# KohakuBlueleaf/UwUDiff

Hardware: AMD Instinct MI355X
Metric: train images/sec (whole node), DiT-S/2 256^2 latent (higher is better)
Workload: dtype bf16; 1 GPU; DiT-S/2 (L12 D384 h6), 4x32x32 synthetic latents + pooled-text cond 1280, eps-MSE, AdamW lr1e-6 wd0.01 cosine; random-init weights; per_gpu_batch=768, global_batch=768, parallelism=dp1

## Files before the change

include/uwu_hip.h:

```cpp
#ifndef UWU_HIP_H
#define UWU_HIP_H

#include <stddef.h>
#include <stdint.h>

#ifdef __cplusplus
extern "C" {
#endif

#define UWU_F32 0
#define UWU_BF16 1

#define UWU_OK 0
#define UWU_EINVAL (-1)
#define UWU_ELAUNCH (-2)
#define UWU_ENOTIMPL (-3)

#define UWU_PT_EPSILON 0
#define UWU_PT_V 1
#define UWU_PT_SAMPLE 2
#define UWU_PT_RF 3

#define UWU_EPI_NONE 0
#define UWU_EPI_BIAS 1
// ... 138 lines not shown
enum {
  UWU_PROF_GEMM_FWD = 0, UWU_PROF_GEMM_DGRAD = 1, UWU_PROF_GEMM_WGRAD = 2, UWU_PROF_GEMM_FC1_GELU = 3,
  UWU_PROF_GEMM_FC2_DGELU = 4, UWU_PROF_ATTN_FWD = 5, UWU_PROF_ATTN_BWD = 6, UWU_PROF_LN_FWD = 7, UWU_PROF_LN_BWD = 8,
  UWU_PROF_CONV = 9, UWU_PROF_OTHER = 10
};
int uwu_prof_enable(int on);
int uwu_prof_collect(int tag, int kind, double* ms, double* flops, double* bytes, int* launches);

int uwu_colsum(const void* X, int dtype, int M, int N, int ldx, float* out, int accumulate, void* stream);

int uwu_skinny_linear_ok(int M, int N, int K);
int uwu_skinny_linear_fwd(const float* X, const float* W, const float* bias, float* Y, float* Y2, int M, int N, int K,
                          int epilogue, void* stream);
int uwu_skinny_linear_dgrad(const float* dY, const float* W, float* dX, int M, int N, int K, void* stream);
int uwu_skinny_linear_wgrad(const float* dY, const float* X, float* dW, float* db, int M, int N, int K, void* stream);
int uwu_colsum_batched(const void* X, int dtype, int batch, int M, int N, int ldx, float* out, int accumulate,
                       void* stream);


int uwu_add_ln_modulate_fwd(const void* x_in, const void* y, const float* gate, const float* shift,
                            const float* scale, int mod_ld, void* x_out, void* h, float* mean, float* rstd,
                            int B, int T, int D, float eps, int affine, int dtype, void* stream);
int uwu_add_ln_modulate_fwd_q8(const void* x_in, const void* y, const float* gate, const float* shift, const float* scale,
                               int mod_ld, void* x_out, void* q8, int ldq, void* q8t, int ldqt, const float* q_scale,
                               float* q_amax, float* mean, float* rstd, int B, int T, int D, float eps, void* stream);


int uwu_add_ln_modulate_bwd(const void* dh, const void* x, const float* mean, const float* rstd,
                            const float* scale, const void* dx_in, const void* y, const float* gate,
                            int mod_ld, void* dx_out, void* dy, float* dshift, float* dscale, float* dgate,
// ... 43 lines not shown
int uwu_attention_rope_fwd(const void* q, const void* k, const void* v, const float* rope_tab, void* o, float* lse, int B,
                           int T, int H, int d, int ldq, int ldk, int ldv, int ldo, int ldt, float scale, int dtype,
                           void* stream);
int uwu_attention_rope_bwd(const void* q, const void* k, const void* v, const float* rope_tab, const void* o, const void* dO,
                           const float* lse, void* dq, void* dk, void* dv, int B, int T, int H, int d, int ldq, int ldk,
                           int ldv, int ldo, int ldt, float scale, int dtype, void* stream);


int uwu_timestep_embedding(const float* t, int B, int dim, float max_period, void* out, int dtype,
                           void* stream);
int uwu_silu_fwd(const void* x, void* y, int64_t n, int dtype, void* stream);
int uwu_silu_bwd(const void* x, const void* dy, void* dx, int64_t n, int dtype, void* stream);

int uwu_add(const void* a, const void* b, void* out, int64_t n, int dtype, void* stream);
int uwu_transpose_bf16(const void* src, void* dst, int rows, int cols, int ld_src, int ld_dst, void* stream);

int uwu_patchify(const float* img, void* tok, int B, int C, int H, int W, int p, int dtype, void* stream);
int uwu_unpatchify(const void* tok, int dtype, float* img, int B, int C, int H, int W, int p, void* stream);
int uwu_add_pos(void* x, const float* pos, int B, int T, int D, int dtype, void* stream);


int uwu_groupnorm_fwd(const void* x, const float* gamma, const float* beta, void* y, float* mean, float* rstd,
                      int B, int HW, int C, int G, float eps, int silu, int dtype, void* stream);
size_t uwu_groupnorm_fwd_det_ws_bytes(int B, int HW, int C, int G);
int uwu_groupnorm_fwd_det(const void* x, const float* gamma, const float* beta, void* y, float* mean, float* rstd, void* ws,
                          size_t ws_bytes, int B, int HW, int C, int G, float eps, int silu, int dtype, void* stream);
int uwu_groupnorm_bwd(const void* dy, const void* x, const float* mean, const float* rstd, const float* gamma,
                      const float* beta, void* dx, float* dgamma, float* dbeta, float* ws, int B, int HW, int C, int G,
                      int silu, int dtype, void* stream);
int uwu_im2col3x3(const void* x, void* col, int B, int H, int W, int C, int stride, int dtype, void* stream);
// ... 46 lines not shown
```

uwudiff_amd/csrc/dit.cpp:

```cpp
#include <hip/hip_runtime.h>
#include <math.h>
#include <stddef.h>
#include <stdint.h>
#include <stdlib.h>

#include "../../include/uwu_hip.h"
#include "env.h"

void uwu_set_error(const char* fmt, ...);

namespace {

constexpr int WGRAD_BLOCKS = 512;

struct Layout {
  size_t es;
  int64_t M, D, D3, D4, Kp, Ko;
  size_t feat, t_pre, t_h, temb, yemb, c, sc, mod;
  size_t sc16, dmod16;
  size_t tok, xe;
  size_t layer0, layer_stride;
  bool ckpt;
  size_t keep, scratch0;
  size_t o_x0, o_m1, o_r1, o_h1, o_qkv, o_lse, o_ao, o_y1, o_x1, o_m2, o_r2, o_h2, o_u, o_f, o_y2;
  size_t o_rope;
  size_t o_h1t, o_aot, o_h2t, o_ft;
  size_t xF, mF, rF, hF, otok;
  size_t dx, dy, dh, dqkv, dao, du, delta, dotok, dmod, dsc, dc, dth, dtp;
  size_t w2t;
  size_t wsc, wsc_bytes;
  size_t x8, x8t, dy8, dy8t, w8, w8_layer;
  size_t total;
};

inline size_t al(size_t x) { return (x + 255) & ~(size_t)255; }

Layout make_layout(const uwu_dit_desc& d) {
  Layout L{};
  L.es = d.dtype == UWU_BF16 ? 2 : 4;
  L.M = (int64_t)d.B * d.T;
  L.D = d.D;
  L.D3 = 3 * (int64_t)d.D;
  L.D4 = (int64_t)d.mlp_ratio * d.D;
  L.Kp = (int64_t)d.in_ch * d.patch * d.patch;
  L.Ko = (int64_t)d.out_ch * d.patch * d.patch;
  size_t p = 0;
  auto take = [&](size_t bytes) { size_t o = p; p = al(p + bytes); return o; };
  const size_t f4 = 4;
  L.feat = take((size_t)d.B * d.freq_dim * f4);
  L.t_pre = take((size_t)d.B * d.D * f4);
// ... 36 lines not shown
  L.layer_stride = L.ckpt ? L.keep : q;
  L.layer0 = p;
  p += (size_t)d.L * L.layer_stride;
  if (L.ckpt) L.scratch0 = take(q);
  L.xF = take(L.M * L.D * L.es);
  L.mF = take(L.M * f4);
  L.rF = take(L.M * f4);
  L.hF = take(L.M * L.D * L.es);
  L.otok = take(L.M * L.Ko * L.es);
  L.dx = take(L.M * L.D * L.es);
  L.dy = take(L.M * L.D * L.es);
  L.dh = take(L.M * L.D * L.es);
  L.dqkv = take(L.M * L.D3 * L.es);
  L.dao = take(L.M * L.D * L.es);
  L.du = take(L.M * L.D4 * L.es);
  L.w2t = take((size_t)L.D4 * d.D * 2);
  L.delta = take((size_t)d.B * d.H * d.T * f4);
  L.dotok = take(L.M * L.Ko * L.es);
  L.dmod = take((size_t)d.B * d.mod_total * f4);
  L.dsc = take((size_t)d.B * d.D * f4);
  L.dc = take((size_t)d.B * d.D * f4);
  L.dth = take((size_t)d.B * d.D * f4);
  L.dtp = take((size_t)d.B * d.D * f4);
  L.wsc_bytes = uwu_gemm_wgrad_scratch_bytes((int)L.D4, d.D, (int)L.M);
  for (const size_t t : {uwu_gemm_wgrad_scratch_bytes(d.D, (int)L.D4, (int)L.M),
                         uwu_gemm_wgrad_scratch_bytes((int)L.D3, d.D, (int)L.M),
                         uwu_gemm_wgrad_scratch_bytes(d.D, d.D, (int)L.M),
                         uwu_gemm_wgrad_pair_scratch_bytes((int)L.D4, d.D, d.D, (int)L.D4, (int)L.M),
                         uwu_gemm_wgrad_pair_scratch_bytes((int)L.D3, d.D, d.D, d.D, (int)L.M)})
    if (t > L.wsc_bytes) L.wsc_bytes = t;
  if (d.fp8) {
// ... 39 lines not shown
    if (d->fp8 < 0 || d->fp8 > 2 || d->dtype != UWU_BF16 || d->D % 128 || d->mlp_ratio != 4 || ((int64_t)d->B * d->T) % 128 ||
        !d->f8_scale || !d->f8_amax || !d->f8_fmt) {
      uwu_set_error("dit: fp8 mode needs bf16 activations, D %% 128 == 0, B*T %% 128 == 0, mlp_ratio 4 and the scale / amax / fmt arrays");
      return UWU_EINVAL;
    }
  }
  return UWU_OK;
}

#define RUN(expr)              \
  do {                         \
    int rc_ = (expr);          \
    if (rc_ != UWU_OK) return rc_; \
  } while (0)

int lin_fwd(const void* X, const void* W, const float* bias, void* Y, void* Y2, int M, int N, int K, int dt, int cdt,
            int epi, void* st) {
  return uwu_gemm(X, W, Y, Y2, bias, nullptr, M, N, K, K, K, N, 0, 0, 0, dt, cdt, epi, 1, st);
}
int lin_fwd32(const float* X, const float* W, const float* bias, float* Y, float* Y2, int M, int N, int K, int epi, void* st) {
  if (M <= 16 && N <= 4096 && uwu_skinny_linear_ok(M, N, K)) return uwu_skinny_linear_fwd(X, W, bias, Y, Y2, M, N, K, epi, st);
  return lin_fwd(X, W, bias, Y, Y2, M, N, K, UWU_F32, UWU_F32, epi, st);
}
int lin_dgrad(const void* dY, const void* W, void* dX, const void* aux, int M, int N, int K, int dt, void* st,
              float* colsum = nullptr) {
  return uwu_gemm(dY, W, dX, colsum, nullptr, aux, M, K, N, N, K, K, K, 0, 1, dt, dt,
                  aux ? UWU_EPI_DGELU : UWU_EPI_NONE, 1, st);
}
static bool mod_bf16(const uwu_dit_desc& d) {
  return d.dtype == UWU_BF16 && d.B >= 64 && d.mod_total % 8 == 0;
}
int lin_dgrad_splitk(const void* dY, const void* W, float* dX, int M, int N, int K, void* st) {
  if (hipMemsetAsync(dX, 0, (size_t)M * K * sizeof(float), (hipStream_t)st) != hipSuccess) {
    uwu_set_error("dgrad_splitk: memset failed");
    return UWU_ELAUNCH;
  }
// ... 20 lines not shown
  if (split > ktiles) split = ktiles;
  if (split < 1) split = 1;
  return uwu_gemm(dY, X, dW, nullptr, nullptr, nullptr, N, K, M, N, K, K, 0, 1, 1, dt, UWU_F32, UWU_EPI_ACCUM, split, st);
}

bool wgrad_pair_ok(int M, int Na, int Ka, int Nb, int Kb, size_t scratch_bytes) {
  const size_t need = uwu_gemm_wgrad_pair_scratch_bytes(Na, Ka, Nb, Kb, M);
  return need && need <= scratch_bytes;
}
int lin_wgrad_pair(const void* dYa, const void* Xa, float* dWa, float* dba, int Na, int Ka, const void* dYb, const void* Xb,
                   float* dWb, float* dbb, int Nb, int Kb, int M, void* st, void* scratch, size_t scratch_bytes) {
  return uwu_gemm_wgrad_pair(dYa, Xa, dWa, dba, Na, Ka, Na, Ka, Ka, dYb, Xb, dWb, dbb, Nb, Kb, Nb, Kb, Kb, M, UWU_BF16,
                             WGRAD_BLOCKS, scratch, scratch_bytes, st);
}

int lin_wgrad32(const float* dY, const float* X, float* dW, float* db, int M, int N, int K, void* st) {
  if (M <= 16 && uwu_skinny_linear_ok(M, N, K)) return uwu_skinny_linear_wgrad(dY, X, dW, db, M, N, K, st);
  RUN(lin_wgrad(dY, X, dW, M, N, K, UWU_F32, st));
  return uwu_colsum(dY, UWU_F32, M, N, N, db, 1, st);
}

struct F8 {
  int mode;
  float* scale;
  float* amax;
  const int32_t* fmt;
  char *x8, *x8t, *dy8, *dy8t, *wsc, *w8;
  size_t wsc_bytes, w8_layer;
  int D;
  void* st;
  int role(int l, int r) const { return 12 * l + r; }
  char* w(int l, int i, bool t) const {
// ... 250 lines not shown
  RUN(uwu_timestep_embedding(t, B, d.freq_dim, 10000.f, P.at(L.feat), UWU_F32, st));
  RUN(lin_fwd32(P.at<float>(L.feat), w32 + d.off_t_w1, w32 + d.off_t_b1, P.at<float>(L.t_pre), P.at<float>(L.t_h), B, D,
                d.freq_dim, UWU_EPI_BIAS_SILU, st));
  RUN(lin_fwd32(P.at<float>(L.t_h), w32 + d.off_t_w2, w32 + d.off_t_b2, P.at<float>(L.temb), nullptr, B, D, D, UWU_EPI_BIAS, st));
  const void* cptr = P.at(L.temb);
  if (cond) {
    RUN(lin_fwd32(cond, w32 + d.off_y_w, w32 + d.off_y_b, P.at<float>(L.yemb), nullptr, B, D, d.cond_dim, UWU_EPI_BIAS, st));
    RUN(uwu_add(P.at(L.temb), P.at(L.yemb), P.at(L.c), (int64_t)B * D, UWU_F32, st));
    cptr = P.at(L.c);
  }
  RUN(uwu_silu_fwd(cptr, P.at(L.sc), (int64_t)B * D, UWU_F32, st));
  if (mod_bf16(d)) {
    RUN(uwu_cast_f32_to_bf16(P.at<float>(L.sc), P.at(L.sc16), (int64_t)B * D, st));
    RUN(lin_fwd(P.at(L.sc16), wb + d.off_mod_w * es, w32 + d.off_mod_b, P.at(L.mod), nullptr, B, ML, D, UWU_BF16, UWU_F32, UWU_EPI_BIAS, st));
  } else {
    RUN(lin_fwd32(P.at<float>(L.sc), w32 + d.off_mod_w, w32 + d.off_mod_b, P.at<float>(L.mod), nullptr, B, ML, D, UWU_EPI_BIAS, st));
  }
  const float* mod = P.at<float>(L.mod);

  const F8 f8{d.fp8, d.f8_scale, d.f8_amax, d.f8_fmt, P.at<char>(L.x8), nullptr, P.at<char>(L.dy8),
              P.at<char>(L.dy8t), P.at<char>(L.wsc), P.at<char>(L.w8), L.wsc_bytes, L.w8_layer, d.D, st};
  if (d.fp8) {
    const F8 fw{2, d.f8_scale, d.f8_amax, d.f8_fmt, nullptr, nullptr, nullptr, nullptr, nullptr, f8.w8, 0, L.w8_layer, d.D, st};
    const int rows[4] = {D3, D, D4, D}, cols[4] = {D, D, D, D4};
    for (int l = 0; l < d.L; ++l) {
      const LayerW w = layer_weights(d, l);
      const void* ws4[4] = {w.qkv_w, w.o_w, w.fc1_w, w.fc2_w};
      for (int i = 0; i < 4; ++i)
        RUN(uwu_fp8_amax(ws4[i], UWU_BF16, (int64_t)rows[i] * cols[i], d.f8_amax + fw.role(l, 8 + i), st));
    }
    RUN(uwu_fp8_update_scales(d.f8_amax, d.f8_scale, d.f8_fmt, 12 * d.L, 1.f, st));
    for (int l = 0; l < d.L; ++l) {
      const LayerW w = layer_weights(d, l);
      const void* ws4[4] = {w.qkv_w, w.o_w, w.fc1_w, w.fc2_w};
      for (int i = 0; i < 4; ++i)
        RUN(fw.quant(ws4[i], UWU_BF16, rows[i], cols[i], fw.role(l, 8 + i), fw.w(l, i, false), fw.w(l, i, true), nullptr, true));
    }
  }

  RUN(uwu_patchify(noisy, P.at(L.tok), B, d.in_ch, d.img, d.img, d.patch, dt, st));
  RUN(lin_fwd(P.at(L.tok), wb + d.off_patch_w * es, w32 + d.off_patch_b, P.lay(0, L.o_x0), nullptr, M, D, (int)L.Kp, dt,
              dt, UWU_EPI_BIAS, st));
  RUN(uwu_add_pos(P.lay(0, L.o_x0), d.pos, B, T, D, dt, st));

  for (int l = 0; l < d.L; ++l) RUN(block_forward(d, L, P, f8, l, false, st));
  {
    const int l = d.L - 1;
    const float* mp = mod + (int64_t)l * 6 * D;
    const float* mf = mod + (int64_t)d.L * 6 * D;
    RUN(uwu_add_ln_modulate_fwd(P.lay(l, L.o_x1), P.lay(l, L.o_y2), mp + 5 * D, mf + 0, mf + D, ML, P.at(L.xF),
                                P.at(L.hF), P.at<float>(L.mF), P.at<float>(L.rF), B, T, D, d.ln_eps, 0, dt, st));
    RUN(lin_fwd(P.at(L.hF), wb + d.off_final_w * es, w32 + d.off_final_b, P.at(L.otok), nullptr, M, (int)L.Ko, D, dt, dt,
                UWU_EPI_BIAS, st));
    RUN(uwu_unpatchify(P.at(L.otok), dt, out, B, d.out_ch, d.img, d.img, d.patch, st));
  }
  return UWU_OK;
}

// ... 15 lines not shown
  if (hipMemsetAsync(dmod, 0, (size_t)B * ML * sizeof(float), (hipStream_t)st) != hipSuccess) {
    uwu_set_error("dit_backward: memset failed");
    return UWU_ELAUNCH;
  }
  const float scale = 1.f / sqrtf((float)(D / d.H));
  const F8 f8{d.fp8, d.f8_scale, d.f8_amax, d.f8_fmt, P.at<char>(L.x8), nullptr, P.at<char>(L.dy8),
              P.at<char>(L.dy8t), P.at<char>(L.wsc), P.at<char>(L.w8), L.wsc_bytes, L.w8_layer, d.D, st};
  Fork fk{static_cast<hipStream_t>(st), {}, {}, false};
  fk.on = d.side_stream && d.side_stream != st && !d.fp8 && dt == UWU_BF16 && M <= 16384 && !L.ckpt &&
          fork_resources(fk, static_cast<hipStream_t>(d.side_stream));
  char* const wsc = P.at<char>(L.wsc);
  bool side_used[4] = {false, false, false, false};
  const bool pairs = !fk.on && !d.fp8 && dt == UWU_BF16 && M > 16384 && !L.ckpt;
  const bool pair_fc = pairs && wgrad_pair_ok(M, D4, D, D, D4, L.wsc_bytes);
  const bool pair_attn = pairs && wgrad_pair_ok(M, D3, D, D, D, L.wsc_bytes);

  RUN(uwu_patchify(dout, P.at(L.dotok), B, d.out_ch, d.img, d.img, d.patch, dt, st));
  RUN(lin_wgrad(P.at(L.dotok), P.at(L.hF), g + d.off_final_w, M, (int)L.Ko, D, dt, st));
  RUN(uwu_colsum(P.at(L.dotok), dt, M, (int)L.Ko, (int)L.Ko, g + d.off_final_b, 1, st));
  RUN(lin_dgrad(P.at(L.dotok), wb + d.off_final_w * es, P.at(L.dh), nullptr, M, (int)L.Ko, D, dt, st));
  {
    const int l = d.L - 1;
    const float* mp = mod + (int64_t)l * 6 * D;
    const float* mf = mod + (int64_t)d.L * 6 * D;
    float* dmp = dmod + (int64_t)l * 6 * D;
    float* dmf = dmod + (int64_t)d.L * 6 * D;
    RUN(uwu_add_ln_modulate_bwd(P.at(L.dh), P.at(L.xF), P.at<float>(L.mF), P.at<float>(L.rF), mf + D, nullptr,
                                P.lay(l, L.o_y2), mp + 5 * D, ML, P.at(L.dx), P.at(L.dy), dmf + 0, dmf + D, dmp + 5 * D,
                                B, T, D, 0, dt, st));
  }
// ... 9 lines not shown
                   f8.role(l, 6), f8.role(l, 2), f8.role(l, 10), f8.x8, f8.dy8t));
      } else {
      RUN(f8_bwd(f8, P.at(L.dy), P.lay(l, L.o_ft), f8.w(l, 3, true), g + w.off_fc2_w, g + w.off_fc2_b, P.at(L.du), P.lay(l, L.o_u),
                 g + w.off_fc1_b, M, D, D4, f8.role(l, 7), f8.role(l, 3), f8.role(l, 11)));
      RUN(f8_bwd(f8, P.at(L.du), P.lay(l, L.o_h2t), f8.w(l, 2, true), g + w.off_fc1_w, nullptr, P.at(L.dh), nullptr, nullptr, M, D4, D,
                 f8.role(l, 6), f8.role(l, 2), f8.role(l, 10)));
      }
    } else {
    if (!pair_fc) {
    RUN(on_side(fk, 0, [&](void* s2, int k) {
      return lin_wgrad(P.at(L.dy), P.lay(l, L.o_f), g + w.off_fc2_w, M, D, D4, dt, s2, wsc + (size_t)k * L.wsc_bytes, L.wsc_bytes, g + w.off_fc2_b);
    }));
    side_used[0] = true;
    }
    if (side_used[1]) RUN(join_side(fk, 1));
    if (dt == UWU_BF16 && D == 384 && M % 256 == 0 && M >= 256 * 256 && D4 % 64 == 0 && D4 >= 1024 && D4 <= 2048) {
      RUN(uwu_transpose_bf16(w.fc2_w, P.at(L.w2t), D, D4, D4, D, st));
      RUN(uwu_gemm(P.at(L.dy), P.at(L.w2t), P.at(L.du), nullptr, nullptr, P.lay(l, L.o_u), M, D4, D, D, D, D4, D4, 0, 0, dt, dt,
                   UWU_EPI_DGELU, 1, st));
    } else {
      RUN(lin_dgrad(P.at(L.dy), w.fc2_w, P.at(L.du), P.lay(l, L.o_u), M, D, D4, dt, st, nullptr));
    }
    if (pair_fc) {
      RUN(lin_wgrad_pair(P.at(L.du), P.lay(l, L.o_h2), g + w.off_fc1_w, g + w.off_fc1_b, D4, D, P.at(L.dy), P.lay(l, L.o_f),
                         g + w.off_fc2_w, g + w.off_fc2_b, D, D4, M, st, wsc, L.wsc_bytes));
    } else {
    RUN(on_side(fk, 1, [&](void* s2, int k) {
      return lin_wgrad(P.at(L.du), P.lay(l, L.o_h2), g + w.off_fc1_w, M, D4, D, dt, s2, wsc + (size_t)k * L.wsc_bytes, L.wsc_bytes, g + w.off_fc1_b);
    }));
    side_used[1] = true;
    }
    RUN(lin_dgrad(P.at(L.du), w.fc1_w, P.at(L.dh), nullptr, M, D4, D, dt, st));
    RUN(join_side(fk, 0));
// ... 75 lines not shown
    RUN(uwu_cast_f32_to_bf16(dmod, P.at(L.dmod16), (int64_t)B * ML, st));
    RUN(lin_wgrad(P.at(L.dmod16), P.at(L.sc16), g + d.off_mod_w, B, ML, D, UWU_BF16, st));
    RUN(uwu_colsum(dmod, UWU_F32, B, ML, ML, g + d.off_mod_b, 1, st));
    if (hipMemsetAsync(P.at(L.dsc), 0, (size_t)B * D * sizeof(float), (hipStream_t)st) != hipSuccess) {
      uwu_set_error("dit_backward: memset failed");
      return UWU_ELAUNCH;
    }
    {
      const int tiles = ((B + 127) / 128) * ((D + 127) / 128), ktiles = (ML + 63) / 64;
      int split = (512 + tiles - 1) / tiles;
      if (split > ktiles) split = ktiles;
      RUN(uwu_gemm(P.at(L.dmod16), wb + d.off_mod_w * es, P.at(L.dsc), nullptr, nullptr, nullptr, B, D, ML, ML, D, D, 0, 0, 1, UWU_BF16,
                   UWU_F32, UWU_EPI_ACCUM, split, st));
    }
  } else {
    RUN(lin_wgrad32(dmod, P.at<float>(L.sc), g + d.off_mod_w, g + d.off_mod_b, B, ML, D, st));
    RUN(lin_dgrad_splitk(dmod, w32 + d.off_mod_w, P.at<float>(L.dsc), B, ML, D, st));
  }
  const void* cptr = d.cond_dim > 0 ? P.at(L.c) : P.at(L.temb);
  RUN(uwu_silu_bwd(cptr, P.at(L.dsc), P.at(L.dc), (int64_t)B * D, UWU_F32, st));
  if (d.cond_dim > 0) {
  }
  RUN(lin_wgrad32(P.at<float>(L.dc), P.at<float>(L.t_h), g + d.off_t_w2, g + d.off_t_b2, B, D, D, st));
  if (B <= 16 && uwu_skinny_linear_ok(B, D, D) && D <= 512) RUN(uwu_skinny_linear_dgrad(P.at<float>(L.dc), w32 + d.off_t_w2, P.at<float>(L.dth), B, D, D, st));
  else RUN(lin_dgrad(P.at(L.dc), w32 + d.off_t_w2, P.at(L.dth), nullptr, B, D, D, UWU_F32, st));
  RUN(uwu_silu_bwd(P.at(L.t_pre), P.at(L.dth), P.at(L.dtp), (int64_t)B * D, UWU_F32, st));
  RUN(lin_wgrad32(P.at<float>(L.dtp), P.at<float>(L.feat), g + d.off_t_w1, g + d.off_t_b1, B, D, d.freq_dim, st));
  return UWU_OK;
}

extern "C" int uwu_dit_backward_cond(const uwu_dit_desc* dp, const float* cond, void* st) {
  RUN(check_desc(dp));
  const uwu_dit_desc& d = *dp;
  if (d.cond_dim <= 0) return UWU_OK;
  if (!cond || !d.g32) { uwu_set_error("dit_backward_cond: null tensor"); return UWU_EINVAL; }
  const Layout L = make_layout(d);
  Ptrs P{static_cast<char*>(d.ws), L};
  return lin_wgrad32(P.at<float>(L.dc), cond, d.g32 + d.off_y_w, d.g32 + d.off_y_b, d.B, d.D, d.cond_dim, st);
}
// ... 1 lines not shown
```

uwudiff_amd/lib.py:

```python
import ctypes
import os
from ctypes import c_char_p, c_float, c_int, c_int32, c_int64, c_size_t, c_void_p

import torch

_HERE = os.path.dirname(os.path.abspath(__file__))
LIB_PATH = os.path.join(_HERE, "libuwu_hip.so")

F32, BF16 = 0, 1
PT = {"epsilon": 0, "v_prediction": 1, "sample": 2, "rectified_flow": 3}
EPI_NONE, EPI_BIAS, EPI_BIAS_GELU, EPI_DGELU, EPI_BIAS_SILU, EPI_ACCUM = 0, 1, 2, 3, 4, 5
ACT = {"quick_gelu": 0, "gelu": 1}
GATE = {"gated-gelu": 0}


class UwuError(RuntimeError):
    pass


class DitDesc(ctypes.Structure):
    _fields_ = (
        [(n, c_int32) for n in ("B", "T", "D", "H", "L", "mlp_ratio", "in_ch", "out_ch", "patch", "img", "dtype",
                                "cond_dim", "freq_dim")]
        + [("ln_eps", c_float), ("mod_total", c_int32)]
# ... 63 lines not shown
                                  P, P]),
    "uwu_gemm_wgrad_scratch_bytes": (ctypes.c_size_t, [c_int, c_int, c_int]),
    "uwu_gemm_wgrad": (c_int, [P, P, P, P] + [c_int] * 8 + [P, ctypes.c_size_t, P]),
    "uwu_gemm_wgrad_pair_scratch_bytes": (ctypes.c_size_t, [c_int] * 5),
    "uwu_gemm_wgrad_pair": (c_int, ([P, P, P, P] + [c_int] * 5) * 2 + [c_int] * 3 + [P, ctypes.c_size_t, P]),
    "uwu_gemm_prof_enable": (c_int, [c_int]),
    "uwu_gemm_prof_collect": (c_int, [c_int, P, P, P]),
    "uwu_prof_enable": (c_int, [c_int]),
    "uwu_prof_collect": (c_int, [c_int, c_int, P, P, P, P]),
    "uwu_colsum": (c_int, [P, c_int, c_int, c_int, c_int, P, c_int, P]),
    "uwu_colsum_batched": (c_int, [P, c_int, c_int, c_int, c_int, c_int, P, c_int, P]),
    "uwu_skinny_linear_ok": (c_int, [c_int, c_int, c_int]),
    "uwu_skinny_linear_fwd": (c_int, [P, P, P, P, P, c_int, c_int, c_int, c_int, P]),
    "uwu_skinny_linear_dgrad": (c_int, [P, P, P, c_int, c_int, c_int, P]),
    "uwu_skinny_linear_wgrad": (c_int, [P, P, P, P, c_int, c_int, c_int, P]),
    "uwu_add_ln_modulate_fwd": (c_int, [P, P, P, P, P, c_int, P, P, P, P, c_int, c_int, c_int, c_float, c_int, c_int, P]),
    "uwu_add_ln_modulate_fwd_q8": (c_int, [P, P, P, P, P, c_int, P, P, c_int, P, c_int, P, P, P, P, c_int, c_int, c_int, c_float, P]),
    "uwu_add_ln_modulate_bwd": (c_int, [P, P, P, P, P, P, P, P, c_int, P, P, P, P, P, c_int, c_int, c_int, c_int, c_int, P]),
    "uwu_attention_fwd": (c_int, [P, P, P, P, P] + [c_int] * 9 + [c_float, c_int, P]),
    "uwu_attention_d512_fwd": (c_int, [P, P, P, P] + [c_int] * 6 + [c_float, c_int, P]),
    "uwu_attention_causal_fwd": (c_int, [P] * 5 + [c_int] * 8 + [c_float, c_int, P]),
    "uwu_text_embed": (c_int, [P, P, P, P, c_int, c_int, c_int, c_int, c_int, P]),
    "uwu_bias_act_fwd": (c_int, [P, P, P, c_int, c_int, c_int, c_int, c_int, P]),
    "uwu_text_pool": (c_int, [P, P, P, c_int, c_int, c_int, c_int, c_int, P]),
    "uwu_attention_relbias_fwd": (c_int, [P] * 6 + [c_int] * 8 + [c_float, c_int, P]),
    "uwu_add_rmsnorm_fwd": (c_int, [P] * 5 + [c_int, c_int, c_float, c_int, P]),
    "uwu_gated_act_fwd": (c_int, [P, P] + [c_int] * 6 + [P]),
    "uwu_t5_rel_bias": (c_int, [P, P, P, c_int, c_int, c_int, P]),
    "uwu_token_embed": (c_int, [P, P, P, c_int, c_int, c_int, c_int, c_int, P]),
    "uwu_attention_bwd": (c_int, [P] * 10 + [c_int] * 9 + [c_float, c_int, P]),
# ... 100 lines not shown
```

Baseline: 17640 images/s.

## Add edge kernels for patch embed, small fp32 linears, and batched fc2 transpose

```diff
diff --git a/include/uwu_hip.h b/include/uwu_hip.h
--- a/include/uwu_hip.h
+++ b/include/uwu_hip.h
@@ -176,6 +176,14 @@
                           int epilogue, void* stream);
 int uwu_skinny_linear_dgrad(const float* dY, const float* W, float* dX, int M, int N, int K, void* stream);
 int uwu_skinny_linear_wgrad(const float* dY, const float* X, float* dW, float* db, int M, int N, int K, void* stream);
+int uwu_edge_patch_ok(int D, int Kp);
+int uwu_edge_patch_fwd(const void* tok, const void* W, const float* bias, const float* pos, void* x0, int B, int T, int D,
+                       int Kp, void* stream);
+int uwu_edge_linear_ok(int M, int N, int K);
+int uwu_edge_linear_fwd(const float* X, const float* W, const float* bias, float* Y, float* Y2, int M, int N, int K,
+                        int epilogue, void* stream);
+int uwu_edge_linear_wgrad(const float* dY, const float* X, float* dW, float* db, int M, int N, int K, void* stream);
+int uwu_edge_linear_dgrad(const float* dY, const float* W, float* dX, int M, int N, int K, void* stream);
 int uwu_colsum_batched(const void* X, int dtype, int batch, int M, int N, int ldx, float* out, int accumulate,
                        void* stream);
 
@@ -249,6 +257,8 @@
 
 int uwu_add(const void* a, const void* b, void* out, int64_t n, int dtype, void* stream);
 int uwu_transpose_bf16(const void* src, void* dst, int rows, int cols, int ld_src, int ld_dst, void* stream);
+int uwu_transpose_bf16_batched(const void* src, void* dst, int rows, int cols, int ld_src, int ld_dst, int batch,
+                               int64_t stride_src, int64_t stride_dst, void* stream);
 
 int uwu_patchify(const float* img, void* tok, int B, int C, int H, int W, int p, int dtype, void* stream);
 int uwu_unpatchify(const void* tok, int dtype, float* img, int B, int C, int H, int W, int p, void* stream);
diff --git a/uwudiff_amd/csrc/dit.cpp b/uwudiff_amd/csrc/dit.cpp
--- a/uwudiff_amd/csrc/dit.cpp
+++ b/uwudiff_amd/csrc/dit.cpp
@@ -27,6 +27,7 @@
   size_t o_h1t, o_aot, o_h2t, o_ft;
   size_t xF, mF, rF, hF, otok;
   size_t dx, dy, dh, dqkv, dao, du, delta, dotok, dmod, dsc, dc, dth, dtp;
+  int w2t_layers;
   size_t w2t;
   size_t wsc, wsc_bytes;
   size_t x8, x8t, dy8, dy8t, w8, w8_layer;
@@ -34,6 +35,10 @@
 };
 
 inline size_t al(size_t x) { return (x + 255) & ~(size_t)255; }
+
+inline bool w2t_shape(const uwu_dit_desc& d, int64_t M, int64_t D4) {
+  return !d.fp8 && d.dtype == UWU_BF16 && d.D == 384 && M % 256 == 0 && M >= 256 * 256 && D4 % 64 == 0 && D4 >= 1024 && D4 <= 2048;
+}
 
 Layout make_layout(const uwu_dit_desc& d) {
   Layout L{};
@@ -100,7 +105,8 @@
   L.dqkv = take(L.M * L.D3 * L.es);
   L.dao = take(L.M * L.D * L.es);
   L.du = take(L.M * L.D4 * L.es);
-  L.w2t = take((size_t)L.D4 * d.D * 2);
+  L.w2t_layers = w2t_shape(d, L.M, L.D4) && !d.checkpoint ? d.L : 1;
+  L.w2t = take((size_t)L.w2t_layers * L.D4 * d.D * 2);
   L.delta = take((size_t)d.B * d.H * d.T * f4);
   L.dotok = take(L.M * L.Ko * L.es);
   L.dmod = take((size_t)d.B * d.mod_total * f4);
@@ -170,12 +176,20 @@
     if (rc_ != UWU_OK) return rc_; \
   } while (0)
 
+inline bool al16(const void* p) { return (reinterpret_cast<uintptr_t>(p) & 15) == 0; }
+static bool edge_on() {
+  static UwuEnv off("UWU_DIT_EDGE");
+  return !off.get().is('0');
+}
+
 int lin_fwd(const void* X, const void* W, const float* bias, void* Y, void* Y2, int M, int N, int K, int dt, int cdt,
             int epi, void* st) {
   return uwu_gemm(X, W, Y, Y2, bias, nullptr, M, N, K, K, K, N, 0, 0, 0, dt, cdt, epi, 1, st);
 }
-int lin_fwd32(const float* X, const float* W, const float* bias, float* Y, float* Y2, int M, int N, int K, int epi, void* st) {
+int lin_fwd32(const float* X, const float* W, const float* bias, float* Y, float* Y2, int M, int N, int K, int epi, void* st,
+              bool rows = true) {
   if (M <= 16 && N <= 4096 && uwu_skinny_linear_ok(M, N, K)) return uwu_skinny_linear_fwd(X, W, bias, Y, Y2, M, N, K, epi, st);
+  if (rows && M > 16 && edge_on() && uwu_edge_linear_ok(M, N, K) && al16(X)) return uwu_edge_linear_fwd(X, W, bias, Y, Y2, M, N, K, epi, st);
   return lin_fwd(X, W, bias, Y, Y2, M, N, K, UWU_F32, UWU_F32, epi, st);
 }
 int lin_dgrad(const void* dY, const void* W, void* dX, const void* aux, int M, int N, int K, int dt, void* st,
@@ -226,8 +240,9 @@
                              WGRAD_BLOCKS, scratch, scratch_bytes, st);
 }
 
-int lin_wgrad32(const float* dY, const float* X, float* dW, float* db, int M, int N, int K, void* st) {
+int lin_wgrad32(const float* dY, const float* X, float* dW, float* db, int M, int N, int K, void* st, bool rows = true) {
   if (M <= 16 && uwu_skinny_linear_ok(M, N, K)) return uwu_skinny_linear_wgrad(dY, X, dW, db, M, N, K, st);
+  if (rows && M > 16 && edge_on() && uwu_edge_linear_ok(M, N, K) && al16(X)) return uwu_edge_linear_wgrad(dY, X, dW, db, M, N, K, st);
   RUN(lin_wgrad(dY, X, dW, M, N, K, UWU_F32, st));
   return uwu_colsum(dY, UWU_F32, M, N, N, db, 1, st);
 }
@@ -508,7 +523,8 @@
     RUN(uwu_cast_f32_to_bf16(P.at<float>(L.sc), P.at(L.sc16), (int64_t)B * D, st));
     RUN(lin_fwd(P.at(L.sc16), wb + d.off_mod_w * es, w32 + d.off_mod_b, P.at(L.mod), nullptr, B, ML, D, UWU_BF16, UWU_F32, UWU_EPI_BIAS, st));
   } else {
-    RUN(lin_fwd32(P.at<float>(L.sc), w32 + d.off_mod_w, w32 + d.off_mod_b, P.at<float>(L.mod), nullptr, B, ML, D, UWU_EPI_BIAS, st));
+    RUN(lin_fwd32(P.at<float>(L.sc), w32 + d.off_mod_w, w32 + d.off_mod_b, P.at<float>(L.mod), nullptr, B, ML, D, UWU_EPI_BIAS, st,
+                  false));
   }
   const float* mod = P.at<float>(L.mod);
 
@@ -533,9 +549,13 @@
   }
 
   RUN(uwu_patchify(noisy, P.at(L.tok), B, d.in_ch, d.img, d.img, d.patch, dt, st));
-  RUN(lin_fwd(P.at(L.tok), wb + d.off_patch_w * es, w32 + d.off_patch_b, P.lay(0, L.o_x0), nullptr, M, D, (int)L.Kp, dt,
-              dt, UWU_EPI_BIAS, st));
-  RUN(uwu_add_pos(P.lay(0, L.o_x0), d.pos, B, T, D, dt, st));
+  if (dt == UWU_BF16 && edge_on() && uwu_edge_patch_ok(D, (int)L.Kp)) {
+    RUN(uwu_edge_patch_fwd(P.at(L.tok), wb + d.off_patch_w * es, w32 + d.off_patch_b, d.pos, P.lay(0, L.o_x0), B, T, D, (int)L.Kp, st));
+  } else {
+    RUN(lin_fwd(P.at(L.tok), wb + d.off_patch_w * es, w32 + d.off_patch_b, P.lay(0, L.o_x0), nullptr, M, D, (int)L.Kp, dt,
+                dt, UWU_EPI_BIAS, st));
+    RUN(uwu_add_pos(P.lay(0, L.o_x0), d.pos, B, T, D, dt, st));
+  }
 
   for (int l = 0; l < d.L; ++l) RUN(block_forward(d, L, P, f8, l, false, st));
   {
@@ -581,6 +601,11 @@
   const bool pairs = !fk.on && !d.fp8 && dt == UWU_BF16 && M > 16384 && !L.ckpt;
   const bool pair_fc = pairs && wgrad_pair_ok(M, D4, D, D, D4, L.wsc_bytes);
   const bool pair_attn = pairs && wgrad_pair_ok(M, D3, D, D, D, L.wsc_bytes);
+
+  const bool w2t_path = w2t_shape(d, M, D4);
+  const bool w2t_once = w2t_path && edge_on() && L.w2t_layers == d.L;
+  if (w2t_once)
+    RUN(uwu_transpose_bf16_batched(layer_weights(d, 0).fc2_w, P.at(L.w2t), D, D4, D4, D, d.L, d.layer_stride, (int64_t)D4 * D, st));
 
   RUN(uwu_patchify(dout, P.at(L.dotok), B, d.out_ch, d.img, d.img, d.patch, dt, st));
   RUN(lin_wgrad(P.at(L.dotok), P.at(L.hF), g + d.off_final_w, M, (int)L.Ko, D, dt, st));
@@ -620,9 +645,10 @@
     side_used[0] = true;
     }
     if (side_used[1]) RUN(join_side(fk, 1));
-    if (dt == UWU_BF16 && D == 384 && M % 256 == 0 && M >= 256 * 256 && D4 % 64 == 0 && D4 >= 1024 && D4 <= 2048) {
-      RUN(uwu_transpose_bf16(w.fc2_w, P.at(L.w2t), D, D4, D4, D, st));
-      RUN(uwu_gemm(P.at(L.dy), P.at(L.w2t), P.at(L.du), nullptr, nullptr, P.lay(l, L.o_u), M, D4, D, D, D, D4, D4, 0, 0, dt, dt,
+    if (w2t_path) {
+      const void* w2t = P.at<char>(L.w2t) + (w2t_once ? (size_t)l * D4 * D * 2 : 0);
+      if (!w2t_once) RUN(uwu_transpose_bf16(w.fc2_w, P.at(L.w2t), D, D4, D4, D, st));
+      RUN(uwu_gemm(P.at(L.dy), w2t, P.at(L.du), nullptr, nullptr, P.lay(l, L.o_u), M, D4, D, D, D, D4, D4, 0, 0, dt, dt,
                    UWU_EPI_DGELU, 1, st));
     } else {
       RUN(lin_dgrad(P.at(L.dy), w.fc2_w, P.at(L.du), P.lay(l, L.o_u), M, D, D4, dt, st, nullptr));
@@ -728,7 +754,7 @@
                    UWU_F32, UWU_EPI_ACCUM, split, st));
     }
   } else {
-    RUN(lin_wgrad32(dmod, P.at<float>(L.sc), g + d.off_mod_w, g + d.off_mod_b, B, ML, D, st));
+    RUN(lin_wgrad32(dmod, P.at<float>(L.sc), g + d.off_mod_w, g + d.off_mod_b, B, ML, D, st, false));
     RUN(lin_dgrad_splitk(dmod, w32 + d.off_mod_w, P.at<float>(L.dsc), B, ML, D, st));
   }
   const void* cptr = d.cond_dim > 0 ? P.at(L.c) : P.at(L.temb);
@@ -737,6 +763,7 @@
   }
   RUN(lin_wgrad32(P.at<float>(L.dc), P.at<float>(L.t_h), g + d.off_t_w2, g + d.off_t_b2, B, D, D, st));
   if (B <= 16 && uwu_skinny_linear_ok(B, D, D) && D <= 512) RUN(uwu_skinny_linear_dgrad(P.at<float>(L.dc), w32 + d.off_t_w2, P.at<float>(L.dth), B, D, D, st));
+  else if (edge_on() && uwu_edge_linear_ok(B, D, D)) RUN(uwu_edge_linear_dgrad(P.at<float>(L.dc), w32 + d.off_t_w2, P.at<float>(L.dth), B, D, D, st));
   else RUN(lin_dgrad(P.at(L.dc), w32 + d.off_t_w2, P.at(L.dth), nullptr, B, D, D, UWU_F32, st));
   RUN(uwu_silu_bwd(P.at(L.t_pre), P.at(L.dth), P.at(L.dtp), (int64_t)B * D, UWU_F32, st));
   RUN(lin_wgrad32(P.at<float>(L.dtp), P.at<float>(L.feat), g + d.off_t_w1, g + d.off_t_b1, B, D, d.freq_dim, st));
diff --git a/uwudiff_amd/csrc/edge.hip b/uwudiff_amd/csrc/edge.hip
--- /dev/null
+++ b/uwudiff_amd/csrc/edge.hip
@@ -0,0 +1,249 @@
+#include "common.h"
+
+namespace {
+
+__device__ __forceinline__ int feat_of_row(int r) { return (r & 16) | ((r & 4) << 1) | ((r & 8) >> 1) | (r & 3); }
+
+template <int NKS, bool POS>
+__global__ void __launch_bounds__(256) edge_patch_fwd_kernel(const bf16_t* __restrict__ tok, const bf16_t* __restrict__ W,
+                                                             const float* __restrict__ bias, const float* __restrict__ pos,
+                                                             bf16_t* __restrict__ x0, int B, int T, int D, int Kp, int bblocks) {
+  const int lane = threadIdx.x & 63, r = lane & 31, h = lane >> 5;
+  const int nwaves = gridDim.x * 4;
+  const int ntiles = T * bblocks, nblocks = (D + 31) >> 5;
+  const int frow = feat_of_row(r);
+  const uint4 zero4 = {0u, 0u, 0u, 0u};
+  for (int tile = blockIdx.x * 4 + (threadIdx.x >> 6); tile < ntiles; tile += nwaves) {
+    const int bb = tile / T, t = tile - bb * T;
+    const int b = bb * 32 + r;
+    const bool live = b < B;
+    const int64_t m = (int64_t)(live ? b : B - 1) * T + t;
+    uint4 tf[NKS];
+#pragma unroll
+    for (int ks = 0; ks < NKS; ++ks) {
+      const int k0 = ks * 16 + 8 * h;
+      tf[ks] = k0 < Kp ? *reinterpret_cast<const uint4*>(tok + m * Kp + k0) : zero4;
+    }
+    for (int nb = 0; nb < nblocks; ++nb) {
+      const int feat = nb * 32 + frow;
+      f32x16 acc;
+#pragma unroll
+      for (int i = 0; i < 16; ++i) acc[i] = 0.f;
+#pragma unroll
+      for (int ks = 0; ks < NKS; ++ks) {
+        const int k0 = ks * 16 + 8 * h;
+        const uint4 wf = (feat < D && k0 < Kp) ? *reinterpret_cast<const uint4*>(W + (int64_t)feat * Kp + k0) : zero4;
+        acc = __builtin_amdgcn_mfma_f32_32x32x16_bf16(*reinterpret_cast<const bf16x8*>(&wf),
+                                                      *reinterpret_cast<const bf16x8*>(&tf[ks]), acc, 0, 0, 0);
+      }
+#pragma unroll
+      for (int g = 0; g < 2; ++g) {
+        const int f0 = nb * 32 + g * 16 + h * 8;
+        if (f0 < D && live) {
+          const f32x8 bv = load8(bias + f0);
+          f32x8 v;
+#pragma unroll
+          for (int j = 0; j < 8; ++j) v[j] = (float)(bf16_t)(acc[8 * g + j] + bv[j]);
+          if (POS) v = v + load8(pos + (int64_t)t * D + f0);
+          store8(x0 + m * D + f0, v);
+        }
+      }
+    }
+  }
+}
+
+enum { LIN_FWD = 0, LIN_WGRAD = 1, LIN_DGRAD = 2 };
+constexpr int LT = 32, LLD = 36;
+
+template <bool TR>
+__device__ __forceinline__ f32x4 lin_tile_load(const float* __restrict__ G, int idx0, int nidx, int c0, int nc, int ld, int tid) {
+  const int a = tid >> 3, q = (tid & 7) * 4;
+  const int gi = TR ? idx0 + a : idx0 + q, gc = TR ? c0 + q : c0 + a;
+  if (gi >= nidx || gc >= nc) return f32x4{0.f, 0.f, 0.f, 0.f};
+  return load4(TR ? G + (int64_t)gi * ld + gc : G + (int64_t)gc * ld + gi);
+}
+template <bool TR>
+__device__ __forceinline__ void lin_tile_store(float (*S)[LLD], f32x4 v, int tid) {
+  const int a = tid >> 3, q = (tid & 7) * 4;
+  if (TR) {
+#pragma unroll
+    for (int e = 0; e < 4; ++e) S[q + e][a] = v[e];
+  } else {
+    *reinterpret_cast<f32x4*>(&S[a][q]) = v;
+  }
+}
+
+template <int MODE, int EPI>
+__global__ void __launch_bounds__(256) edge_lin32_kernel(const float* __restrict__ A, const float* __restrict__ Bm,
+                                                         const float* __restrict__ bias, float* __restrict__ C,
+                                                         float* __restrict__ C2, float* __restrict__ db, int NI, int NJ,
+                                                         int NCn, int lda, int ldb, int ldc) {
+  constexpr bool TA = MODE != LIN_WGRAD, TB = MODE == LIN_FWD;
+  __shared__ __attribute__((aligned(16))) float As[LT][LLD];
+  __shared__ __attribute__((aligned(16))) float Bs[LT][LLD];
+  const int tid = threadIdx.x, ty = tid >> 4, tx = tid & 15;
+  const int i0 = blockIdx.y * LT, j0 = blockIdx.x * LT;
+  const bool colsum = MODE == LIN_WGRAD && db && blockIdx.x == 0;
+  f32x4 pa = lin_tile_load<TA>(A, i0, NI, 0, NCn, lda, tid), pb = lin_tile_load<TB>(Bm, j0, NJ, 0, NCn, ldb, tid);
+  f32x2 acc0 = {0.f, 0.f}, acc1 = {0.f, 0.f}, asum = {0.f, 0.f};
+  for (int c0 = 0; c0 < NCn; c0 += LT) {
+    lin_tile_store<TA>(As, pa, tid);
+    lin_tile_store<TB>(Bs, pb, tid);
+    __syncthreads();
+    if (c0 + LT < NCn) {
+      pa = lin_tile_load<TA>(A, i0, NI, c0 + LT, NCn, lda, tid);
+      pb = lin_tile_load<TB>(Bm, j0, NJ, c0 + LT, NCn, ldb, tid);
+    }
+#pragma unroll 8
+    for (int c = 0; c < LT; ++c) {
+      const f32x2 a = *reinterpret_cast<const f32x2*>(&As[c][2 * ty]);
+      const f32x2 b = *reinterpret_cast<const f32x2*>(&Bs[c][2 * tx]);
+      acc0 += f32x2{a[0], a[0]} * b;
+      acc1 += f32x2{a[1], a[1]} * b;
+      if (colsum) asum += a;
+    }
+    __syncthreads();
+  }
+  const int j = j0 + 2 * tx;
+  if (j >= NJ) return;
+#pragma unroll
+  for (int r = 0; r < 2; ++r) {
+    const int i = i0 + 2 * ty + r;
+    if (i >= NI) break;
+    f32x2 v = r ? acc1 : acc0;
+    float* cp = C + (int64_t)i * ldc + j;
+    if (MODE == LIN_FWD) {
+      if (EPI != UWU_EPI_NONE) v += *reinterpret_cast<const f32x2*>(bias + j);
+      *reinterpret_cast<f32x2*>(cp) = v;
+      if (EPI == UWU_EPI_BIAS_SILU) *reinterpret_cast<f32x2*>(C2 + (int64_t)i * ldc + j) = f32x2{silu_f(v[0]), silu_f(v[1])};
+    } else if (MODE == LIN_WGRAD) {
+      *reinterpret_cast<f32x2*>(cp) = *reinterpret_cast<const f32x2*>(cp) + v;
+      if (colsum && tx == 0) db[i] += asum[r];
+    } else {
+      *reinterpret_cast<f32x2*>(cp) = v;
+    }
+  }
+}
+
+__global__ void __launch_bounds__(256) transpose_bf16_batched_kernel(const bf16_t* __restrict__ src, bf16_t* __restrict__ dst,
+                                                                     int rows, int cols, int lds, int ldd, int64_t stride_src,
+                                                                     int64_t stride_dst) {
+  __shared__ bf16_t tile[32][34];
+  const int tx = threadIdx.x & 31, ty = threadIdx.x >> 5;
+  const int r0 = blockIdx.y * 32, c0 = blockIdx.x * 32;
+  src += blockIdx.z * stride_src;
+  dst += blockIdx.z * stride_dst;
+#pragma unroll
+  for (int k = 0; k < 4; ++k) {
+    const int r = r0 + ty + 8 * k, c = c0 + tx;
+    tile[ty + 8 * k][tx] = (r < rows && c < cols) ? src[(int64_t)r * lds + c] : (bf16_t)0.f;
+  }
+  __syncthreads();
+#pragma unroll
+  for (int k = 0; k < 4; ++k) {
+    const int c = c0 + ty + 8 * k, r = r0 + tx;
+    if (c < cols && r < rows) dst[(int64_t)c * ldd + r] = tile[tx][ty + 8 * k];
+  }
+}
+
+bool aligned16(const void* p) { return (reinterpret_cast<uintptr_t>(p) & 15) == 0; }
+
+}
+
+extern "C" int uwu_edge_patch_ok(int D, int Kp) { return D >= 8 && D % 8 == 0 && Kp >= 8 && Kp <= 64 && Kp % 8 == 0; }
+
+extern "C" int uwu_edge_patch_fwd(const void* tok, const void* W, const float* bias, const float* pos, void* x0, int B, int T,
+                                  int D, int Kp, void* stream) {
+  UWU_CHECK_ARG(tok && W && bias && x0 && B > 0 && T > 0, "edge_patch_fwd: null pointer or empty batch");
+  UWU_CHECK_ARG(uwu_edge_patch_ok(D, Kp), "edge_patch_fwd: D=%d Kp=%d not covered", D, Kp);
+  UWU_CHECK_ARG(aligned16(tok) && aligned16(W) && aligned16(bias) && aligned16(pos) && aligned16(x0),
+                "edge_patch_fwd: pointers must be 16-byte aligned");
+  UWU_CHECK_ARG((int64_t)B * T < (1ll << 31), "edge_patch_fwd: too many tokens");
+  hipStream_t st = (hipStream_t)stream;
+  const int bblocks = (B + 31) / 32;
+  const int64_t tiles = (int64_t)T * bblocks;
+  UWU_CHECK_ARG(tiles < (1ll << 31), "edge_patch_fwd: too many tiles");
+  const int grid = (int)((tiles + 3) / 4 < 2048 ? (tiles + 3) / 4 : 2048);
+  UwuProfScope prof(stream);
+#define EP(NKS, POS)                                                                                                       \
+  hipLaunchKernelGGL((edge_patch_fwd_kernel<NKS, POS>), dim3(grid), dim3(256), 0, st, (const bf16_t*)tok, (const bf16_t*)W, \
+                     bias, pos, (bf16_t*)x0, B, T, D, Kp, bblocks)
+#define EP_K(POS)                     \
+  do {                                \
+    if (Kp <= 16) EP(1, POS);         \
+    else if (Kp <= 32) EP(2, POS);    \
+    else if (Kp <= 48) EP(3, POS);    \
+    else EP(4, POS);                  \
+  } while (0)
+  if (pos) EP_K(true);
+  else EP_K(false);
+#undef EP_K
+#undef EP
+  const double M = (double)B * T;
+  prof.done(UWU_PROF_OTHER, 0, 2.0 * M * D * Kp, M * Kp * 2 + M * D * 2 + (double)D * Kp * 2);
+  UWU_LAUNCH_CHECK("edge_patch_fwd");
+  return UWU_OK;
+}
+
+extern "C" int uwu_edge_linear_ok(int M, int N, int K) { return M >= 1 && N >= 4 && K >= 4 && N % 4 == 0 && K % 4 == 0; }
+
+extern "C" int uwu_edge_linear_fwd(const float* X, const float* W, const float* bias, float* Y, float* Y2, int M, int N, int K,
+                                   int epilogue, void* stream) {
+  UWU_CHECK_ARG(X && W && Y, "edge_linear_fwd: null pointer");
+  UWU_CHECK_ARG(uwu_edge_linear_ok(M, N, K), "edge_linear_fwd: M=%d N=%d K=%d not covered", M, N, K);
+  UWU_CHECK_ARG(epilogue == UWU_EPI_NONE || epilogue == UWU_EPI_BIAS || epilogue == UWU_EPI_BIAS_SILU,
+                "edge_linear_fwd: epilogue %d", epilogue);
+  UWU_CHECK_ARG(epilogue == UWU_EPI_NONE || bias, "edge_linear_fwd: bias missing");
+  UWU_CHECK_ARG(epilogue != UWU_EPI_BIAS_SILU || Y2, "edge_linear_fwd: second output missing");
+  UWU_CHECK_ARG(aligned16(X) && aligned16(W) && aligned16(Y) && aligned16(Y2) && aligned16(bias),
+                "edge_linear_fwd: pointers must be 16-byte aligned");
+  hipStream_t st = (hipStream_t)stream;
+  const dim3 grid((N + LT - 1) / LT, (M + LT - 1) / LT);
+  UwuProfScope prof(stream);
+#define EL(EPI)                                                                                                             \
+  hipLaunchKernelGGL((edge_lin32_kernel<LIN_FWD, EPI>), grid, dim3(256), 0, st, X, W, bias, Y, Y2, (float*)nullptr, M, N, K, K, \
+                     K, N)
+  if (epilogue == UWU_EPI_NONE) EL(UWU_EPI_NONE);
+  else if (epilogue == UWU_EPI_BIAS) EL(UWU_EPI_BIAS);
+  else EL(UWU_EPI_BIAS_SILU);
+#undef EL
+  prof.done(UWU_PROF_GEMM_FWD, 1, 2.0 * M * N * K, ((double)N * K + (double)M * K + (double)M * N) * 4);
+  UWU_LAUNCH_CHECK("edge_linear_fwd");
+  return UWU_OK;
+}
+
+extern "C" int uwu_edge_linear_wgrad(const float* dY, const float* X, float* dW, float* db, int M, int N, int K, void* stream) {
+  UWU_CHECK_ARG(dY && X && dW, "edge_linear_wgrad: null pointer");
+  UWU_CHECK_ARG(uwu_edge_linear_ok(M, N, K), "edge_linear_wgrad: M=%d N=%d K=%d not covered", M, N, K);
+  UWU_CHECK_ARG(aligned16(dY) && aligned16(X) && aligned16(dW), "edge_linear_wgrad: pointers must be 16-byte aligned");
+  const dim3 grid((K + LT - 1) / LT, (N + LT - 1) / LT);
+  UwuProfScope prof(stream);
+  hipLaunchKernelGGL((edge_lin32_kernel<LIN_WGRAD, UWU_EPI_NONE>), grid, dim3(256), 0, (hipStream_t)stream, dY, X,
+                     (const float*)nullptr, dW, (float*)nullptr, db, N, K, M, N, K, K);
+  prof.done(UWU_PROF_GEMM_WGRAD, 1, 2.0 * M * N * K, ((double)N * K * 2 + (double)M * K + (double)M * N) * 4);
+  UWU_LAUNCH_CHECK("edge_linear_wgrad");
+  return UWU_OK;
+}
+
+extern "C" int uwu_edge_linear_dgrad(const float* dY, const float* W, float* dX, int M, int N, int K, void* stream) {
+  UWU_CHECK_ARG(dY && W && dX, "edge_linear_dgrad: null pointer");
+  UWU_CHECK_ARG(uwu_edge_linear_ok(M, N, K), "edge_linear_dgrad: M=%d N=%d K=%d not covered", M, N, K);
+  UWU_CHECK_ARG(aligned16(dY) && aligned16(W) && aligned16(dX), "edge_linear_dgrad: pointers must be 16-byte aligned");
+  const dim3 grid((K + LT - 1) / LT, (M + LT - 1) / LT);
+  UwuProfScope prof(stream);
+  hipLaunchKernelGGL((edge_lin32_kernel<LIN_DGRAD, UWU_EPI_NONE>), grid, dim3(256), 0, (hipStream_t)stream, dY, W,
+                     (const float*)nullptr, dX, (float*)nullptr, (float*)nullptr, M, K, N, N, K, K);
+  prof.done(UWU_PROF_GEMM_DGRAD, 1, 2.0 * M * N * K, ((double)N * K + (double)M * K + (double)M * N) * 4);
+  UWU_LAUNCH_CHECK("edge_linear_dgrad");
+  return UWU_OK;
+}
+
+extern "C" int uwu_transpose_bf16_batched(const void* src, void* dst, int rows, int cols, int ld_src, int ld_dst, int batch,
+                                          int64_t stride_src, int64_t stride_dst, void* stream) {
+  UWU_CHECK_ARG(src && dst && rows > 0 && cols > 0 && ld_src >= cols && ld_dst >= rows && batch > 0 && batch <= 65535,
+                "transpose_bf16_batched: bad argument");
+  hipLaunchKernelGGL(transpose_bf16_batched_kernel, dim3((cols + 31) / 32, (rows + 31) / 32, batch), dim3(256), 0,
+                     (hipStream_t)stream, (const bf16_t*)src, (bf16_t*)dst, rows, cols, ld_src, ld_dst, stride_src, stride_dst);
+  UWU_LAUNCH_CHECK("transpose_bf16_batched");
+  return UWU_OK;
+}
diff --git a/uwudiff_amd/lib.py b/uwudiff_amd/lib.py
--- a/uwudiff_amd/lib.py
+++ b/uwudiff_amd/lib.py
@@ -101,6 +101,13 @@
     "uwu_skinny_linear_fwd": (c_int, [P, P, P, P, P, c_int, c_int, c_int, c_int, P]),
     "uwu_skinny_linear_dgrad": (c_int, [P, P, P, c_int, c_int, c_int, P]),
     "uwu_skinny_linear_wgrad": (c_int, [P, P, P, P, c_int, c_int, c_int, P]),
+    "uwu_edge_patch_ok": (c_int, [c_int, c_int]),
+    "uwu_edge_patch_fwd": (c_int, [P, P, P, P, P, c_int, c_int, c_int, c_int, P]),
+    "uwu_edge_linear_ok": (c_int, [c_int, c_int, c_int]),
+    "uwu_edge_linear_fwd": (c_int, [P, P, P, P, P, c_int, c_int, c_int, c_int, P]),
+    "uwu_edge_linear_wgrad": (c_int, [P, P, P, P, c_int, c_int, c_int, P]),
+    "uwu_edge_linear_dgrad": (c_int, [P, P, P, c_int, c_int, c_int, P]),
+    "uwu_transpose_bf16_batched": (c_int, [P, P, c_int, c_int, c_int, c_int, c_int, c_int64, c_int64, P]),
     "uwu_add_ln_modulate_fwd": (c_int, [P, P, P, P, P, c_int, P, P, P, P, c_int, c_int, c_int, c_float, c_int, c_int, P]),
     "uwu_add_ln_modulate_fwd_q8": (c_int, [P, P, P, P, P, c_int, P, P, c_int, P, c_int, P, P, P, P, c_int, c_int, c_int, c_float, P]),
     "uwu_add_ln_modulate_bwd": (c_int, [P, P, P, P, P, P, P, P, c_int, P, P, P, P, P, c_int, c_int, c_int, c_int, c_int, P]),
```

New measurement: 17720 images/s, median of 6. About the same (+0.5%).
